# lmb-freiburg/hand3d

Hardware: NVIDIA H100
Metric: images/sec full pipeline 320x320 (higher is better)
Workload: dtype bf16 hi/lo split x3 MMA passes, fp32 accumulate (fp32 parity, 1e-3)

## Files before the change

### hand3d_b200/csrc/common.cuh

```cuda
#pragma once
#include <cuda_runtime.h>
#include <cuda_bf16.h>
#include <cuda_fp16.h>
#include <stdint.h>
#include <stdio.h>
#include <algorithm>
#include <cmath>
#include <string>
#include <vector>

#include "../../include/hand3d_b200.h"

namespace h3d {

void set_error(const char* fmt, ...);
int cuda_fail(cudaError_t e, const char* what, const char* file, int line);

#define H3D_CUDA(expr)                                                     \
    do {                                                                   \
        cudaError_t _e = (expr);                                           \
        if (_e != cudaSuccess) return h3d::cuda_fail(_e, #expr, __FILE__, __LINE__); \
    } while (0)

extern thread_local int64_t t_launches;
// ... 190 lines not shown
    int passes;
    float corr_scale = 0.f;
    Half16 half;
    int pool = 0;
    int* err_flag = nullptr;
    const int* count = nullptr;
};
struct TcTuning {
    int bn = 0;
    int chunk_kb = 0;
    int no_side_stream = 0, no_pool_fusion = 0, lift_direct = 0;
    int c3_ffma = 0;
    int no_seg_fusion = 0;
    int fc_chain = 1;
    int pdl = 1;
};
TcTuning& tc_tuning();
int tc_set_tuning(const char* key, int value);
struct FcLayerDesc {
    Split x; int x_stride, in_features;
    Split w; const float* bias; int out_features, out_pad;
    const float* w_scale = nullptr;
    Split y; int y_stride;
    float* yf; int yf_stride;
    int leaky;
};
struct FcChainDesc { FcLayerDesc layer[4]; int num_layers = 0; };
struct FcChainPlan;
FcChainPlan* fc_chain_plan_create(const FcChainDesc* chains, int num_chains, int B, Half16 half, const float* can, const float* uxyz,
                                  unsigned int* counter, int* err_flag);
void fc_chain_plan_destroy(FcChainPlan* p);
int fc_chain_launch(const FcChainPlan* p, const float* hand_side, float* rot, float* out, cudaStream_t s);
TcConvPlan* tc_conv_plan_create(const TcConvDesc& d, int* rc = nullptr);
void tc_conv_plan_destroy(TcConvPlan* p);
int tc_conv_launch(const TcConvPlan* p, cudaStream_t s);
int64_t tc_conv_flops(const TcConvPlan* p);
int tc_num_sms();
void tc_conv_geometry(int B, int H, int W, int Cout_pad, int pool, int passes, int out[4]);

int launch_pack_conv_w(const float* w_hwio, const float* bias, Split out, float* bias_pad, float* w_scale, int k, int Cin, int Cout,
                       int Cin_pad, int Cout_pad, bool dgrad, Half16 half, cudaStream_t s);
int conv_grad_prep_blocks(int64_t pixels, int64_t* pixels_per_block);
int launch_conv_grad_prep(const float* dy, const float* y, Split out, float* db_part, int B, int H, int W, int Cout, int Cout_pad,
                          int stride, int leaky, cudaStream_t s);
int launch_bias_grad_reduce(const float* db_part, int nblk, int Cout, int Cout_pad, float* db, cudaStream_t s);
struct WgradDesc {
    Split x;
    Split dy;
    int B, H, W, Cin, Cout, Cin_pad, Cout_pad, k, passes;
    float* partial;
    float* dw;
    int* err_flag;
};
// ... 32 lines not shown
```

### hand3d_b200/csrc/conv_wgmma.cu

```cuda
#include <cuda.h>

#include <algorithm>
#include <cstdlib>
#include <cstring>
#include <vector>

#include "common.cuh"
#include "split_fmt.cuh"
#include "wgmma_common.cuh"

namespace h3d {

namespace {

constexpr int BM = 128;
constexpr int BK = 64;
constexpr int kThreads = 384;
constexpr int kConsumerThreads = 256;
constexpr int A_TILE_BYTES = BM * BK * 2;
constexpr int STG_COLS = 64;
constexpr int STG_PITCH = STG_COLS + 1;
constexpr int STG_BYTES = BM * STG_PITCH * 4;
constexpr int kSmemBudget = 227 * 1024 - 2048 - STG_BYTES;

__host__ __device__ constexpr int stage_bytes(int BN, int PASSES) { return (PASSES >= 3 ? 2 : 1) * (A_TILE_BYTES + BN * BK * 2); }
__host__ __device__ constexpr int num_stages(int BN, int PASSES) {
    return kSmemBudget / stage_bytes(BN, PASSES) > 8 ? 8 : kSmemBudget / stage_bytes(BN, PASSES);
}
__host__ __device__ constexpr int smem_bytes(int BN, int PASSES) { return num_stages(BN, PASSES) * stage_bytes(BN, PASSES) + STG_BYTES + 2048; }

struct TcParams {
    const float* bias;
    uint16_t* y_hi; uint16_t* y_lo; uint8_t* y_l8; uint8_t* y_h8; int Cy_total, cy_off;
    float corr_scale;
    float* yf; int Cyf_total, cyf_off;
    int B, H, W, k, pad, cin_chunks;
    int TW, TH, TB, tiles_w, tiles_h, n_tiles, num_tiles;
    int n_valid;
    int pool;
    int chunk_kb;
    int leaky;
    int* err_flag;
    const float* w_scale;
    const int* count;
};

__device__ __forceinline__ int counted_images(const TcParams& p) { return p.count ? min(*p.count, p.B) : p.B; }
__device__ __forceinline__ int counted_tiles(const TcParams& p, int nb) {
    return p.count ? min(p.num_tiles, (nb + p.TB - 1) / p.TB * p.tiles_w * p.tiles_h * p.n_tiles) : p.num_tiles;
}

template <int PASSES, bool FP16, bool SMEM_SCALE = false>
__device__ __forceinline__ void epilogue_store32(const TcParams& p, const float* a, int64_t pix, int n, bool valid, const float* w_scale) {
    float f[32];
    const float4* bp = reinterpret_cast<const float4*>(p.bias + n);
#pragma unroll
    for (int q = 0; q < 8; ++q) {
        const float4 bv = __ldg(bp + q);
        if (PASSES == 4) {
            f[4 * q + 0] = fmaf(a[4 * q + 0], p.corr_scale, bv.x);
            f[4 * q + 1] = fmaf(a[4 * q + 1], p.corr_scale, bv.y);
            f[4 * q + 2] = fmaf(a[4 * q + 2], p.corr_scale, bv.z);
            f[4 * q + 3] = fmaf(a[4 * q + 3], p.corr_scale, bv.w);
        } else if (FP16) {
            const float4 sv = SMEM_SCALE ? reinterpret_cast<const float4*>(w_scale + n)[q] : __ldg(reinterpret_cast<const float4*>(w_scale + n) + q);
            f[4 * q + 0] = fmaf(a[4 * q + 0], sv.x, bv.x);
            f[4 * q + 1] = fmaf(a[4 * q + 1], sv.y, bv.y);
            f[4 * q + 2] = fmaf(a[4 * q + 2], sv.z, bv.z);
// ... 1 lines not shown
        } else {
            f[4 * q + 0] = a[4 * q + 0] + bv.x;
            f[4 * q + 1] = a[4 * q + 1] + bv.y;
            f[4 * q + 2] = a[4 * q + 2] + bv.z;
            f[4 * q + 3] = a[4 * q + 3] + bv.w;
        }
    }
    if (p.leaky) {
#pragma unroll
        for (int q = 0; q < 32; ++q) f[q] = fmaxf(f[q], kNegSlope * f[q]);
    }
    if (p.pool == 1) {
#pragma unroll
        for (int q = 0; q < 32; ++q) {
            f[q] = fmaxf(f[q], __shfl_xor_sync(0xFFFFFFFFu, f[q], 1));
            f[q] = fmaxf(f[q], __shfl_xor_sync(0xFFFFFFFFu, f[q], p.TW));
        }
    }
    if (!valid) return;
    if (n + 32 > p.n_valid) {
        const int cnt = p.n_valid - n;
        if (p.yf && cnt > 0) {
            float* dst = p.yf + pix * p.Cyf_total + p.cyf_off + n;
#pragma unroll
            for (int q = 0; q < 32; ++q)
                if (q < cnt) dst[q] = f[q];
        }
#pragma unroll
        for (int q = 0; q < 32; ++q)
            if (q >= cnt) f[q] = 0.f;
    } else if (p.yf) {
// ... 75 lines not shown
        if (PASSES == 3) {
            tma_load_4d(x_lo, st + A_TILE_BYTES, fb, a0, a1, a2, a3);
            tma_load_2d(w_lo, st + 2 * A_TILE_BYTES + C::B_TILE_BYTES, fb, kcol, n0);
        }
        if (PASSES == 4) {
            tma_load_4d(x_lo, st + A_TILE_BYTES, fb, a0, a1, a2, a3);
            tma_load_4d(x_h8, st + A_TILE_BYTES + C::A8_TILE_BYTES, fb, a0, a1, a2, a3);
            tma_load_2d(w_lo, st + 2 * A_TILE_BYTES + C::B_TILE_BYTES, fb, kcol, n0);
            tma_load_2d(w_l8, st + 2 * A_TILE_BYTES + C::B_TILE_BYTES + C::B8_TILE_BYTES, fb, kcol, n0);
        }
    }
    __syncwarp();
    if (++r.stage == C::STAGES) { r.stage = 0; r.phase ^= 1; }
}

template <int BN, int PASSES, bool FP16>
__device__ __forceinline__ void mma_tile(Ring& r, int kblocks, int chunk_kb, float* racc, int wg, int lane, int* err_flag) {
    using C = RingCfg<BN, PASSES>;
    constexpr int NR = BN / 2;
    constexpr int NR8 = PASSES == 4 ? NR : 1;
    float acc[NR], acc8[NR8];
#pragma unroll
    for (int i = 0; i < NR; ++i) acc[i] = 0.f;
#pragma unroll
    for (int i = 0; i < NR8; ++i) acc8[i] = 0.f;
    for (int kb0 = 0; kb0 < kblocks; kb0 += chunk_kb) {
        const int kb1 = min(kblocks, kb0 + chunk_kb);
        int pend = -1;
        for (int kb = kb0; kb < kb1; ++kb) {
            mbar_wait(&r.full[r.stage], r.phase, err_flag, 3);
            H3D_SKEW(SKEW_CONSUMER, kb);
            const uint32_t sa = smem_u32(r.base + r.stage * C::STAGE_BYTES);
            const uint32_t a_rows = (uint32_t)wg * 64 * 128;
            const uint64_t a_hi = desc_sw128(sa + a_rows);
            const uint64_t a_lo = desc_sw128(sa + A_TILE_BYTES + a_rows);
            const uint64_t b_hi = desc_sw128(sa + (PASSES >= 3 ? 2 : 1) * A_TILE_BYTES);
            const uint64_t b_lo = desc_sw128(sa + 2 * A_TILE_BYTES + C::B_TILE_BYTES);
            fence_regs<NR>(acc);
            fence_regs<NR8>(acc8);
            wgmma_fence();
#pragma unroll
            for (int j = 0; j < BK / 16; ++j) {
                const uint64_t koff = (uint64_t)j * 2;
                mma16<BN, FP16>(acc, a_hi + koff, b_hi + koff, (uint32_t)((kb > kb0) | (j != 0)));
                if (PASSES == 3) {
                    mma16<BN, FP16>(acc, a_hi + koff, b_lo + koff, 1u);
                    mma16<BN, FP16>(acc, a_lo + koff, b_hi + koff, 1u);
                }
            }
            if (PASSES == 4) {
                const uint32_t a8_rows = (uint32_t)wg * 64 * 64;
                const uint64_t a_l8 = desc_sw64(sa + A_TILE_BYTES + a8_rows);
// ... 2 lines not shown
                const uint64_t b_l8 = desc_sw64(sa + 2 * A_TILE_BYTES + C::B_TILE_BYTES + C::B8_TILE_BYTES);
#pragma unroll
                for (int j = 0; j < 2; ++j) {
                    const uint64_t koff = (uint64_t)j * 2;
                    mma8<BN>(acc8, a_l8 + koff, b_h8 + koff, (uint32_t)((kb > kb0) | (j != 0)));
                    mma8<BN>(acc8, a_h8 + koff, b_l8 + koff, 1u);
                }
            }
            wgmma_commit();
            fence_regs<NR>(acc);
            fence_regs<NR8>(acc8);
            H3D_SKEW(SKEW_COMMIT, kb);
            wgmma_wait<1>();
            if (pend >= 0 && lane == 0) mbar_arrive(&r.empty[pend]);
            pend = r.stage;
            if (++r.stage == C::STAGES) { r.stage = 0; r.phase ^= 1; }
        }
        wgmma_wait<0>();
        if (lane == 0) mbar_arrive(&r.empty[pend]);
        fence_regs<NR>(acc);
        fence_regs<NR8>(acc8);
        if constexpr (PASSES == 4) {
#pragma unroll
            for (int i = 0; i < NR; ++i) acc[i] += acc8[i];
        }
        if (kb0 == 0) {
#pragma unroll
            for (int i = 0; i < NR; ++i) racc[i] = acc[i];
        } else {
#pragma unroll
            for (int i = 0; i < NR; ++i) racc[i] += acc[i];
        }
    }
}

template <int BN, int PASSES, bool FP16, class PixOf, bool SMEM_SCALE = false>
__device__ __forceinline__ void store_tile(const TcParams& p, const float* racc, float* stg, int ct, int n0, PixOf pix_of,
                                           const float* w_scale) {
    const int wg = ct >> 7, tt = ct & 127;
    const int r0 = wg * 64 + (tt >> 5) * 16 + ((tt & 31) >> 2);
    const int cq = 2 * (tt & 3);
    const int row = ct & 127, half = ct >> 7;
    int64_t pix; bool valid;
    pix_of(row, pix, valid);
#pragma unroll
    for (int rnd = 0; rnd < BN / STG_COLS; ++rnd) {
        H3D_SKEW(SKEW_EPILOGUE, 2 * rnd);
        named_bar_sync(1, kConsumerThreads);
#pragma unroll
        for (int j = 0; j < STG_COLS / 8; ++j) {
            const int jj = rnd * (STG_COLS / 8) + j, c = 8 * j + cq;
            stg[r0 * STG_PITCH + c] = racc[4 * jj];
            stg[r0 * STG_PITCH + c + 1] = racc[4 * jj + 1];
            stg[(r0 + 8) * STG_PITCH + c] = racc[4 * jj + 2];
            stg[(r0 + 8) * STG_PITCH + c + 1] = racc[4 * jj + 3];
        }
        named_bar_sync(1, kConsumerThreads);
        H3D_SKEW(SKEW_EPILOGUE, 2 * rnd + 1);
        float f[32];
#pragma unroll
        for (int q = 0; q < 32; ++q) f[q] = stg[row * STG_PITCH + half * 32 + q];
        epilogue_store32<PASSES, FP16, SMEM_SCALE>(p, f, pix, n0 + rnd * STG_COLS + half * 32, valid, w_scale);
    }
}

constexpr int kProducerRegs = 40, kConsumerRegs = 232;

template <int BN, int PASSES, bool FP16>
__global__ void __launch_bounds__(kThreads, 1)
conv_tc_kernel(const __grid_constant__ CUtensorMap map_x_hi, const __grid_constant__ CUtensorMap map_x_lo,
               const __grid_constant__ CUtensorMap map_w_hi, const __grid_constant__ CUtensorMap map_w_lo,
               const __grid_constant__ CUtensorMap map_x_h8, const __grid_constant__ CUtensorMap map_w_l8, const TcParams p) {
    using C = RingCfg<BN, PASSES>;
    static_assert(PASSES != 4 || FP16, "fp8-correction mode uses an fp16 main plane");
    static_assert(smem_bytes(BN, PASSES) <= 227 * 1024, "conv_tc_kernel: shared memory budget");

    extern __shared__ __align__(1024) uint8_t smem_raw[];
    uint8_t* smem = reinterpret_cast<uint8_t*>((reinterpret_cast<uintptr_t>(smem_raw) + 1023) & ~(uintptr_t)1023);
    float* stg = reinterpret_cast<float*>(smem + C::STAGES * C::STAGE_BYTES);
    uint64_t* bars = reinterpret_cast<uint64_t*>(smem + C::STAGES * C::STAGE_BYTES + STG_BYTES);
    Ring ring{smem, bars, bars + C::STAGES, 0, 0};

    const int warp = threadIdx.x >> 5, lane = threadIdx.x & 31;
    const int wg = __shfl_sync(0xFFFFFFFFu, (int)threadIdx.x / 128, 0);
    const int kblocks = p.k * p.k * p.cin_chunks;

    if (threadIdx.x == 0) {
        prefetch_tmap(&map_x_hi); prefetch_tmap(&map_w_hi);
        if (PASSES >= 3) { prefetch_tmap(&map_x_lo); prefetch_tmap(&map_w_lo); }
        if (PASSES == 4) { prefetch_tmap(&map_x_h8); prefetch_tmap(&map_w_l8); }
        for (int s = 0; s < C::STAGES; ++s) { mbar_init(&ring.full[s], 1); mbar_init(&ring.empty[s], kConsumerThreads / 32); }
        asm volatile("fence.mbarrier_init.release.cluster;" ::: "memory");
    }
    __syncthreads();
    pdl_launch_dependents();
    H3D_SKEW(SKEW_PDL_TAIL, 0);
    pdl_wait();
    const int nb = counted_images(p), num_tiles = counted_tiles(p, nb);

    if (wg == 0) {
        setmaxnreg_dec<kProducerRegs>();
        if (warp == 0) {
            for (int tile = blockIdx.x; tile < num_tiles; tile += gridDim.x) {
                const int nt = tile % p.n_tiles, mt = tile / p.n_tiles;
                const int tw = mt % p.tiles_w, th = (mt / p.tiles_w) % p.tiles_h, tb = mt / (p.tiles_w * p.tiles_h);
                const int w0 = tw * p.TW - p.pad, h0 = th * p.TH - p.pad, b0 = tb * p.TB, n0 = nt * BN;
                int kcol = 0;
                for (int kh = 0; kh < p.k; ++kh)
                    for (int kw = 0; kw < p.k; ++kw)
                        for (int cc = 0; cc < p.cin_chunks; ++cc, kcol += BK)
                            produce_kblock<BN, PASSES>(ring, &map_x_hi, &map_x_lo, &map_x_h8, &map_w_hi, &map_w_lo, &map_w_l8, cc * BK,
                                                       w0 + kw, h0 + kh, b0, kcol, n0, p.err_flag);
            }
        }
    } else {
        setmaxnreg_inc<kConsumerRegs>();
        const int ct = threadIdx.x - 128;
        float racc[BN / 2];
        for (int tile = blockIdx.x; tile < num_tiles; tile += gridDim.x) {
            const int nt = tile % p.n_tiles, mt = tile / p.n_tiles;
            const int tw = mt % p.tiles_w, th = (mt / p.tiles_w) % p.tiles_h, tb = mt / (p.tiles_w * p.tiles_h);
            mma_tile<BN, PASSES, FP16>(ring, kblocks, p.chunk_kb, racc, ct >> 7, lane, p.err_flag);
            store_tile<BN, PASSES, FP16>(p, racc, stg, ct, nt * BN, [&](int row, int64_t& pix, bool& valid) {
                const int w_l = row % p.TW, h_l = (row / p.TW) % p.TH, b_l = row / (p.TW * p.TH);
                const int w = tw * p.TW + w_l, h = th * p.TH + h_l, b = tb * p.TB + b_l;
                valid = (w < p.W) && (h < p.H) && (b < nb);
                pix = ((int64_t)b * p.H + h) * p.W + w;
                if (p.pool) {
                    const int par = p.pool == 2 ? 1 : 0;
                    valid = valid && ((w & 1) == par) && ((h & 1) == par);
                    pix = ((int64_t)b * (p.H >> 1) + (h >> 1)) * (p.W >> 1) + (w >> 1);
                }
            }, p.w_scale);
        }
    }
}

constexpr int C3_TW = 16, C3_TH = 8;
constexpr int C3T_THREADS = 256;
constexpr int C3T_B_BYTES = 128 * BK * 2;
constexpr int C3T_PW = C3_TW + 2, C3T_PH = C3_TH + 2;
constexpr int C3T_PATCH_FLOATS = C3T_PH * C3T_PW * 3;
constexpr int C3T_SMEM = C3T_B_BYTES + 2 * A_TILE_BYTES + STG_BYTES + C3T_PATCH_FLOATS * 4 + 64 * 4 + 1024 ;

template <bool FP16, bool COUNTED>
__global__ void __launch_bounds__(C3T_THREADS, 2)
conv_c3_tc_kernel(const float* __restrict__ x, const float* __restrict__ w, const TcParams p, const int* __restrict__ slots) {
    extern __shared__ __align__(1024) uint8_t smem_raw[];
    uint8_t* smem = reinterpret_cast<uint8_t*>((reinterpret_cast<uintptr_t>(smem_raw) + 1023) & ~(uintptr_t)1023);
    uint8_t* bsm = smem;
// ... 78 lines not shown
        for (int j = 0; j < 2; ++j) {
            const uint64_t koff = (uint64_t)j * 2;
            mma16<64, FP16>(acc, a_hi + koff, b_hi + koff, (uint32_t)(j != 0));
            mma16<64, FP16>(acc, a_hi + koff, b_lo + koff, 1u);
            mma16<64, FP16>(acc, a_lo + koff, b_hi + koff, 1u);
        }
        wgmma_commit();
        H3D_SKEW(SKEW_COMMIT, tile);
        wgmma_wait<0>();
        fence_regs<32>(acc);
        auto pix_of = [&](int row, int64_t& pix, bool& valid) {
            const int wx = tw * C3_TW + row % C3_TW, hy = th * C3_TH + row / C3_TW;
            valid = (wx < p.W) && (hy < p.H);
            pix = ((int64_t)b * p.H + hy) * p.W + wx;
        };
        if (p.y_lo) store_tile<64, 3, FP16, decltype(pix_of), true>(p, acc, stg, t, 0, pix_of, w_scale);
        else store_tile<64, 1, FP16, decltype(pix_of), true>(p, acc, stg, t, 0, pix_of, w_scale);
    }
}

constexpr int kFcMaxLayers = 4;
constexpr int kFcCluster = 8;
struct FcLayer {
    CUtensorMap map_x_hi, map_x_lo, map_w_hi, map_w_lo;
    TcParams p;
    int kblocks, m_tiles, n_tiles, pad_;
};
struct FcChain { FcLayer layer[kFcMaxLayers]; int num_layers; int pad_[3]; };
struct FcChainParams {
    FcChain chain[2];
    int num_chains, B;
    const float* can; const float* uxyz; const float* hand_side;
// ... 48 lines not shown
            for (int item = rank; item < items; item += kFcCluster) {
                const int nt = item % L.n_tiles, mt = item / L.n_tiles;
                for (int kb = 0; kb < L.kblocks; ++kb)
                    produce_kblock<BN, PASSES>(ring, &L.map_x_hi, &L.map_x_lo, &L.map_x_hi, &L.map_w_hi, &L.map_w_lo, &L.map_w_hi, kb * BK, 0, 0,
                                               mt * BM, kb * BK, nt * BN, P.err_flag);
            }
        } else if (wg >= 1) {
            const int ct = threadIdx.x - 128;
            float racc[BN / 2];
            for (int item = rank; item < items; item += kFcCluster) {
                const int nt = item % L.n_tiles, mt = item / L.n_tiles;
                mma_tile<BN, PASSES, FP16>(ring, L.kblocks, kChunk, racc, ct >> 7, lane, P.err_flag);
                store_tile<BN, PASSES, FP16>(L.p, racc, stg, ct, nt * BN, [&](int row, int64_t& pix, bool& valid) {
                    pix = (int64_t)mt * BM + row;
                    valid = pix < P.B;
                }, L.p.w_scale);
            }
        }
        fc_layer_sync(l);
    }

    if (P.num_chains == 2 && rank == 0) {
        H3D_SKEW(SKEW_TICKET, 0);
        if (threadIdx.x == 0) {
            __threadfence();
            s_last = atomicAdd(P.counter, 1u) == 1u;
            if (s_last) *P.counter = 0u;
        }
        __syncthreads();
        if (s_last) {
            __threadfence();
// ... 41 lines not shown

bool encode_act_map(CUtensorMap* m, const void* base, int C_total, int C_used, int W, int H, int B, int TW, int TH, int TB, int es) {
    EncodeTiledFn fn = get_encode_fn();
    if (!fn) return false;
    cuuint64_t dims[4] = {(cuuint64_t)C_used, (cuuint64_t)W, (cuuint64_t)H, (cuuint64_t)B};
    cuuint64_t strides[3] = {(cuuint64_t)C_total * es, (cuuint64_t)W * C_total * es, (cuuint64_t)H * W * C_total * es};
    cuuint32_t box[4] = {(cuuint32_t)BK, (cuuint32_t)TW, (cuuint32_t)TH, (cuuint32_t)TB};
    cuuint32_t estr[4] = {1, 1, 1, 1};
    CUresult r = fn(m, es == 2 ? CU_TENSOR_MAP_DATA_TYPE_UINT16 : CU_TENSOR_MAP_DATA_TYPE_UINT8, 4, const_cast<void*>(base), dims, strides,
                    box, estr, CU_TENSOR_MAP_INTERLEAVE_NONE, es == 2 ? CU_TENSOR_MAP_SWIZZLE_128B : CU_TENSOR_MAP_SWIZZLE_64B,
                    CU_TENSOR_MAP_L2_PROMOTION_L2_256B, CU_TENSOR_MAP_FLOAT_OOB_FILL_NONE);
    if (r != CUDA_SUCCESS) { set_error("cuTensorMapEncodeTiled(activations) failed: %d", (int)r); return false; }
    return true;
}

bool encode_w_map(CUtensorMap* m, const void* base, int Ktot, int Cout_pad, int BN, int es) {
    EncodeTiledFn fn = get_encode_fn();
    if (!fn) return false;
    cuuint64_t dims[2] = {(cuuint64_t)Ktot, (cuuint64_t)Cout_pad};
    cuuint64_t strides[1] = {(cuuint64_t)Ktot * es};
    cuuint32_t box[2] = {(cuuint32_t)BK, (cuuint32_t)BN};
    cuuint32_t estr[2] = {1, 1};
    CUresult r = fn(m, es == 2 ? CU_TENSOR_MAP_DATA_TYPE_UINT16 : CU_TENSOR_MAP_DATA_TYPE_UINT8, 2, const_cast<void*>(base), dims, strides,
                    box, estr, CU_TENSOR_MAP_INTERLEAVE_NONE, es == 2 ? CU_TENSOR_MAP_SWIZZLE_128B : CU_TENSOR_MAP_SWIZZLE_64B,
                    CU_TENSOR_MAP_L2_PROMOTION_L2_256B, CU_TENSOR_MAP_FLOAT_OOB_FILL_NONE);
    if (r != CUDA_SUCCESS) { set_error("cuTensorMapEncodeTiled(weights) failed: %d", (int)r); return false; }
    return true;
}

namespace {

void choose_tile(int B, int H, int W, int* TW, int* TH, int* TB, bool pool = false) {
    static const int cand[][3] = {{16, 8, 1}, {8, 16, 1}, {32, 4, 1}, {4, 32, 1}, {64, 2, 1}, {128, 1, 1}, {8, 8, 2},
                                  {16, 4, 2}, {4, 16, 2}, {8, 4, 4}, {4, 8, 4}, {4, 4, 8}, {8, 2, 8}, {2, 2, 32}, {1, 1, 128}};
    int64_t best = -1;
    for (auto& c : cand) {
        if (pool && !((c[0] % 2) == 0 && c[0] <= 16 && (c[1] % 2) == 0)) continue;
        const int64_t tiles = (int64_t)ceil_div(W, c[0]) * ceil_div(H, c[1]) * ceil_div(B, c[2]);
        if (best < 0 || tiles < best) { best = tiles; *TW = c[0]; *TH = c[1]; *TB = c[2]; }
    }
}

template <int BN, int PASSES, bool FP16>
int launch_inst(const TcConvPlan* pl, cudaStream_t s);

}

struct TcConvPlan {
    int device = 0;
    TcConvDesc d;
    CUtensorMap map_x_hi, map_x_lo, map_w_hi, map_w_lo, map_x_h8, map_w_l8;
    TcParams p;
    int BN, grid;
};

constexpr int kMaxDevices = 64;
static int current_device() { int dev = 0; if (cudaGetDevice(&dev) != cudaSuccess) { cudaGetLastError(); dev = 0; } return dev; }
int tc_num_sms() {
    static int n[kMaxDevices] = {};
    const int dev = current_device() % kMaxDevices;
    if (!n[dev]) {
        int v = 0;
        if (cudaDeviceGetAttribute(&v, cudaDevAttrMultiProcessorCount, dev) != cudaSuccess || v <= 0) { cudaGetLastError(); v = 132; }
        n[dev] = v;
    }
    return n[dev];
}
template <typename K>
// ... 60 lines not shown
}
#endif

int tc_set_tuning(const char* key, int value) {
    TcTuning& t = tc_tuning();
    const std::string k(key ? key : "");
    if (k == "tc_bn") t.bn = value;
    else if (k == "tc_chunk_kb") t.chunk_kb = value;
    else if (k == "no_side_stream") t.no_side_stream = value;
    else if (k == "no_pool_fusion") t.no_pool_fusion = value;
    else if (k == "lift_direct") t.lift_direct = value;
    else if (k == "c3_ffma") t.c3_ffma = value;
    else if (k == "pdl") t.pdl = value;
    else if (k == "fc_chain") t.fc_chain = value;
    else if (k == "no_seg_fusion") t.no_seg_fusion = value;
#ifdef H3D_SKEW_BUILD
    else if (k.compare(0, 5, "skew_") == 0) return skew_set(key, value);
#endif
    else { set_error("h3d_set_tuning: unknown key '%s'", k.c_str()); return H3D_EINVAL; }
    return H3D_OK;
}

namespace {
int choose_bn(int H, int W, int Cout_pad, int passes) {
    const TcTuning& tune = tc_tuning();
    int BN = Cout_pad % 128 == 0 ? 128 : 64;
    if ((int64_t)H * W <= 256) BN = 64;
    if ((tune.bn == 64 || tune.bn == 128) && Cout_pad % tune.bn == 0) BN = tune.bn;
    if (passes == 4) BN = 64;
    return BN;
}

template <int BN, int PASSES, bool FP16>
int launch_inst(const TcConvPlan* pl, cudaStream_t s) {
    constexpr int smem = smem_bytes(BN, PASSES);
    static bool attr[kMaxDevices] = {};
    if (int rc = smem_opt_in(conv_tc_kernel<BN, PASSES, FP16>, smem, attr)) return rc;
    H3D_CUDA(launch_pdl(conv_tc_kernel<BN, PASSES, FP16>, dim3(pl->grid), dim3(kThreads), smem, s, pl->map_x_hi, pl->map_x_lo, pl->map_w_hi,
                        pl->map_w_lo, pl->map_x_h8, pl->map_w_l8, pl->p));
    return H3D_OK;
}
}

TcConvPlan* tc_conv_plan_create(const TcConvDesc& d, int* rc) {
    int rc_local;
    if (!rc) rc = &rc_local;
    *rc = H3D_EINVAL;
    if (d.Cin_pad % BK != 0 || d.Cout_pad % 64 != 0 || (d.k != 1 && d.k != 3 && d.k != 5 && d.k != 7) || (d.passes != 1 && d.passes != 3 && d.passes != 4)) {
        set_error("tc_conv: unsupported geometry (Cin_pad=%d Cout_pad=%d k=%d passes=%d)", d.Cin_pad, d.Cout_pad, d.k, d.passes);
        return nullptr;
    }
    const bool padded_out = d.Cout % 32 != 0;
    if (d.y.hi && ((d.Cy_total % 8) || (d.cy_off % 8))) { set_error("tc_conv: split output channel offset/stride must be multiples of 8"); return nullptr; }
    if (d.yf && !padded_out && ((d.Cyf_total % 4) || (d.cyf_off % 4))) { set_error("tc_conv: fp32 output channel offset/stride must be multiples of 4"); return nullptr; }
// ... 25 lines not shown
    p.yf = d.yf; p.Cyf_total = d.Cyf_total; p.cyf_off = d.cyf_off;
    p.B = d.B; p.H = d.H; p.W = d.W; p.k = d.k; p.pad = d.k / 2; p.cin_chunks = d.Cin_pad / BK;
    p.TW = TW; p.TH = TH; p.TB = TB;
    p.tiles_w = ceil_div(d.W, TW); p.tiles_h = ceil_div(d.H, TH);
    p.n_tiles = d.Cout_pad / BN;
    p.num_tiles = p.tiles_w * p.tiles_h * ceil_div(d.B, TB) * p.n_tiles;
    p.leaky = d.leaky;
    p.n_valid = d.Cout;
    p.pool = d.pool;
    p.err_flag = d.err_flag;
    p.w_scale = d.w_scale;
    p.count = d.count;
    p.chunk_kb = d.passes >= 3 ? 9 : 27;
    if (tune.chunk_kb > 0) p.chunk_kb = tune.chunk_kb;
    pl->grid = std::min(p.num_tiles, tc_num_sms());
    const int Ktot = d.k * d.k * d.Cin_pad;
    bool ok = encode_act_map(&pl->map_x_hi, d.x.hi, d.Cin_total, d.Cin_pad, d.W, d.H, d.B, TW, TH, TB) &&
              encode_w_map(&pl->map_w_hi, d.w.hi, Ktot, d.Cout_pad, BN);
    if (ok && d.passes == 3)
        ok = encode_act_map(&pl->map_x_lo, d.x.lo, d.Cin_total, d.Cin_pad, d.W, d.H, d.B, TW, TH, TB) &&
             encode_w_map(&pl->map_w_lo, d.w.lo, Ktot, d.Cout_pad, BN);
    if (ok && d.passes == 4)
        ok = encode_act_map(&pl->map_x_lo, d.x.l8, d.Cin_total, d.Cin_pad, d.W, d.H, d.B, TW, TH, TB, 1) &&
             encode_act_map(&pl->map_x_h8, d.x.h8, d.Cin_total, d.Cin_pad, d.W, d.H, d.B, TW, TH, TB, 1) &&
             encode_w_map(&pl->map_w_lo, d.w.h8, Ktot, d.Cout_pad, BN, 1) &&
             encode_w_map(&pl->map_w_l8, d.w.l8, Ktot, d.Cout_pad, BN, 1);
    if (ok && d.passes == 1) { pl->map_x_lo = pl->map_x_hi; pl->map_w_lo = pl->map_w_hi; }
    if (ok && d.passes != 4) { pl->map_x_h8 = pl->map_x_hi; pl->map_w_l8 = pl->map_w_hi; }
    if (!ok) { delete pl; return nullptr; }
    *rc = H3D_OK;
    return pl;
}

void tc_conv_plan_destroy(TcConvPlan* p) { delete p; }

void tc_conv_geometry(int B, int H, int W, int Cout_pad, int pool, int passes, int out[4]) {
    choose_tile(B, H, W, &out[0], &out[1], &out[2], pool == 1);
    out[3] = choose_bn(H, W, Cout_pad, passes);
}

int64_t tc_conv_flops(const TcConvPlan* p) {
    return 2ll * p->d.B * p->d.H * p->d.W * p->d.k * p->d.k * (int64_t)p->d.Cin_pad * p->d.Cout_pad;
}

int tc_conv_launch(const TcConvPlan* pl, cudaStream_t s) {
    const bool fp16 = pl->d.half == Half16::FP16;
    const int key = pl->BN * 10 + pl->d.passes;
#define CASE(BN_, P_)                                                                  \
    case BN_ * 10 + P_:                                                                \
        return fp16 ? launch_inst<BN_, P_, true>(pl, s) : launch_inst<BN_, P_, false>(pl, s);
    switch (key) {
        CASE(64, 1) CASE(64, 3) CASE(128, 1) CASE(128, 3)
        case 64 * 10 + 4: return launch_inst<64, 4, true>(pl, s);
    }
#undef CASE
    set_error("tc_conv: no kernel instance for BN=%d passes=%d", pl->BN, pl->d.passes);
    return H3D_EINVAL;
}

int launch_conv_c3_tc(const float* x, const float* w, const float* bias, Split y, int Cs_total, int cs_off, int B, int H, int W, int leaky,
                      Half16 half, cudaStream_t s, int* err_flag, const int* count, const int* slots) {
    H3D_REQUIRE(x && w && bias && y.hi && !y.l8 && (Cs_total % 8) == 0 && (cs_off % 8) == 0, "conv_c3_tc: bad argument");
    TcParams p{};
    p.bias = bias;
    p.y_hi = y.hi; p.y_lo = y.lo; p.Cy_total = Cs_total; p.cy_off = cs_off;
    p.corr_scale = 1.f;
    p.B = B; p.H = H; p.W = W; p.k = 3; p.pad = 1; p.cin_chunks = 1;
    p.TW = C3_TW; p.TH = C3_TH; p.TB = 1;
// ... 72 lines not shown
```

### hand3d_b200/runtime.py

```python
from __future__ import annotations

import ctypes as C

import numpy as np
import torch

from . import _lib
from ._lib import PRECISIONS, VARIANTS


def _ptr(t):
    return C.c_void_p(0 if t is None else t.data_ptr())


def _stream():
    return C.c_void_p(torch.cuda.current_stream().cuda_stream)


def _chk_f32(t, name, ndim=None):
    if not isinstance(t, torch.Tensor):
        raise TypeError("%s must be a torch.Tensor" % name)
    if not t.is_cuda:
        raise RuntimeError("%s must live on a CUDA device (hand3d_b200 has no CPU path)" % name)
    if t.dtype != torch.float32:
# ... 1080 lines not shown
        B = self.B
        self.center = self.buffer[_lib.TRACK_CENTER * B:(_lib.TRACK_CENTER + 2) * B].view(B, 2)
        self.scale = self.buffer[_lib.TRACK_SCALE * B:(_lib.TRACK_SCALE + 1) * B]
        self.score = self.buffer[_lib.TRACK_SCORE * B:(_lib.TRACK_SCORE + 1) * B]
        self.lost = self.buffer[_lib.TRACK_LOST * B:(_lib.TRACK_LOST + 1) * B].view(torch.int32)
        self.reset()

    def reset(self):
        self.center.fill_(160.0)
        self.scale.fill_(float(np.float32(256.0) / (np.float32(100.0) * np.float32(1.25))))
        self.score.fill_(float("nan"))
        self.lost.fill_(1)


def conv2d_tc_geometry(B, H, W, Cout, pool=0, precision="bf16x3"):
    out = (C.c_int * 4)()
    _lib.check(_lib.load().h3d_conv2d_tc_geometry(B, H, W, Cout, int(pool), PRECISIONS[precision], out), "h3d_conv2d_tc_geometry")
    return tuple(out)


def conv2d_wgrad_geometry(B, H, W, ksize, Cin, Cout):
    out = (C.c_int * 6)()
    _lib.check(_lib.load().h3d_conv2d_wgrad_geometry(B, H, W, ksize, Cin, Cout, out), "h3d_conv2d_wgrad_geometry")
    return tuple(out)


def conv2d_f32_geometry(B, H, W, Cin, Cout, ksize, stride=1, Cin_total=None, cin_off=0, Cout_total=None, cout_off=0, yf=True,
                        planes=None, Cs_total=None, cs_off=0, x_aligned=True, splitk_scratch_floats=_lib.CONV_SPLITK_SCRATCH_FLOATS):
    out = (C.c_int * 6)()
    _lib.check(_lib.load().h3d_conv2d_f32_geometry(
        B, H, W, Cin, Cin if Cin_total is None else Cin_total, cin_off, Cout, Cout if Cout_total is None else Cout_total, cout_off,
# ... 24 lines not shown
```

Measured before the change: 1259.

## Feed conv activations as one TMA row box reused across kernel columns

Adds a row-box feed path to the implicit-GEMM conv kernel. For each kernel row it loads one wide activation box (TW+k-1 columns) and reuses it for all k horizontal taps by offsetting the smem descriptor, while weights stream through a separate ring. The goal is fewer activation TMA loads and less duplicated smem traffic for k>=3 layers with a single 64-channel input chunk. In exchange the pixel ordering within a tile changes (h-major), the pooling shuffle offset changes, and a second barrier ring plus a runtime-sized smem layout are added.

```diff
diff --git a/hand3d_b200/csrc/common.cuh b/hand3d_b200/csrc/common.cuh
--- a/hand3d_b200/csrc/common.cuh
+++ b/hand3d_b200/csrc/common.cuh
@@ -228,6 +228,7 @@
     int no_seg_fusion = 0;
     int fc_chain = 1;
     int pdl = 1;
+    int feed = 0;
 };
 TcTuning& tc_tuning();
 int tc_set_tuning(const char* key, int value);
@@ -250,7 +251,7 @@
 int tc_conv_launch(const TcConvPlan* p, cudaStream_t s);
 int64_t tc_conv_flops(const TcConvPlan* p);
 int tc_num_sms();
-void tc_conv_geometry(int B, int H, int W, int Cout_pad, int pool, int passes, int out[4]);
+void tc_conv_geometry(int B, int H, int W, int Cout_pad, int pool, int passes, int out[5]);
 
 int launch_pack_conv_w(const float* w_hwio, const float* bias, Split out, float* bias_pad, float* w_scale, int k, int Cin, int Cout,
                        int Cin_pad, int Cout_pad, bool dgrad, Half16 half, cudaStream_t s);
diff --git a/hand3d_b200/csrc/conv_wgmma.cu b/hand3d_b200/csrc/conv_wgmma.cu
--- a/hand3d_b200/csrc/conv_wgmma.cu
+++ b/hand3d_b200/csrc/conv_wgmma.cu
@@ -28,6 +28,9 @@
     return kSmemBudget / stage_bytes(BN, PASSES) > 8 ? 8 : kSmemBudget / stage_bytes(BN, PASSES);
 }
 __host__ __device__ constexpr int smem_bytes(int BN, int PASSES) { return num_stages(BN, PASSES) * stage_bytes(BN, PASSES) + STG_BYTES + 2048; }
+constexpr int kRowSlots = 2;
+constexpr int kMaxWStages = 8;
+__host__ __device__ constexpr int wstage_bytes(int BN, int PASSES) { return (PASSES >= 3 ? 2 : 1) * BN * BK * 2; }
 
 struct TcParams {
     const float* bias;
@@ -43,6 +46,7 @@
     int* err_flag;
     const float* w_scale;
     const int* count;
+    int box_bytes, w_stages, wg_rows;
 };
 
 __device__ __forceinline__ int counted_images(const TcParams& p) { return p.count ? min(*p.count, p.B) : p.B; }
@@ -51,7 +55,8 @@
 }
 
 template <int PASSES, bool FP16, bool SMEM_SCALE = false>
-__device__ __forceinline__ void epilogue_store32(const TcParams& p, const float* a, int64_t pix, int n, bool valid, const float* w_scale) {
+__device__ __forceinline__ void epilogue_store32(const TcParams& p, const float* a, int64_t pix, int n, bool valid, int pool_xor,
+                                                 const float* w_scale) {
     float f[32];
     const float4* bp = reinterpret_cast<const float4*>(p.bias + n);
 #pragma unroll
@@ -83,7 +88,7 @@
 #pragma unroll
         for (int q = 0; q < 32; ++q) {
             f[q] = fmaxf(f[q], __shfl_xor_sync(0xFFFFFFFFu, f[q], 1));
-            f[q] = fmaxf(f[q], __shfl_xor_sync(0xFFFFFFFFu, f[q], p.TW));
+            f[q] = fmaxf(f[q], __shfl_xor_sync(0xFFFFFFFFu, f[q], pool_xor));
         }
     }
     if (!valid) return;
@@ -189,28 +194,88 @@
     if (++r.stage == C::STAGES) { r.stage = 0; r.phase ^= 1; }
 }
 
-template <int BN, int PASSES, bool FP16>
-__device__ __forceinline__ void mma_tile(Ring& r, int kblocks, int chunk_kb, float* racc, int wg, int lane, int* err_flag) {
+struct RowFeed {
+    Ring a;
+    int k, box_bytes, w_stages;
+    uint32_t wg_off, kw_off;
+};
+
+template <int PASSES>
+__device__ __forceinline__ void produce_box(RowFeed& f, const CUtensorMap* x_hi, const CUtensorMap* x_lo, int h, int w, int b, int* err_flag) {
+    Ring& r = f.a;
+    mbar_wait(&r.empty[r.stage], r.phase ^ 1, err_flag, 1);
+    H3D_SKEW(SKEW_PRODUCER, r.stage + r.phase * kRowSlots);
+    if (elect_one()) {
+        uint8_t* st = r.base + r.stage * (PASSES == 3 ? 2 : 1) * f.box_bytes;
+        uint64_t* fb = &r.full[r.stage];
+        mbar_expect_tx(fb, (PASSES == 3 ? 2 : 1) * f.box_bytes);
+        tma_load_4d(x_hi, st, fb, 0, h, w, b);
+        if (PASSES == 3) tma_load_4d(x_lo, st + f.box_bytes, fb, 0, h, w, b);
+    }
+    __syncwarp();
+    if (++r.stage == kRowSlots) { r.stage = 0; r.phase ^= 1; }
+}
+
+template <int BN, int PASSES>
+__device__ __forceinline__ void produce_wblock(Ring& r, int w_stages, const CUtensorMap* w_hi, const CUtensorMap* w_lo, int kcol, int n0,
+                                               int* err_flag) {
     using C = RingCfg<BN, PASSES>;
+    mbar_wait(&r.empty[r.stage], r.phase ^ 1, err_flag, 1);
+    H3D_SKEW(SKEW_PRODUCER, r.stage + r.phase * w_stages);
+    if (elect_one()) {
+        uint8_t* st = r.base + r.stage * wstage_bytes(BN, PASSES);
+        uint64_t* fb = &r.full[r.stage];
+        mbar_expect_tx(fb, wstage_bytes(BN, PASSES));
+        tma_load_2d(w_hi, st, fb, kcol, n0);
+        if (PASSES == 3) tma_load_2d(w_lo, st + C::B_TILE_BYTES, fb, kcol, n0);
+    }
+    __syncwarp();
+    if (++r.stage == w_stages) { r.stage = 0; r.phase ^= 1; }
+}
+
+template <int BN, int PASSES, bool FP16, bool ROW_BOX = false>
+__device__ __forceinline__ void mma_tile(Ring& r, int kblocks, int chunk_kb, float* racc, int wg, int lane, int* err_flag,
+                                         RowFeed* f = nullptr) {
+    using C = RingCfg<BN, PASSES>;
+    static_assert(!ROW_BOX || PASSES != 4, "the row-box feed has 16-bit planes only");
     constexpr int NR = BN / 2;
     constexpr int NR8 = PASSES == 4 ? NR : 1;
+    const int stages = ROW_BOX ? f->w_stages : C::STAGES;
     float acc[NR], acc8[NR8];
 #pragma unroll
     for (int i = 0; i < NR; ++i) acc[i] = 0.f;
 #pragma unroll
     for (int i = 0; i < NR8; ++i) acc8[i] = 0.f;
+    int kw = 0;
     for (int kb0 = 0; kb0 < kblocks; kb0 += chunk_kb) {
         const int kb1 = min(kblocks, kb0 + chunk_kb);
-        int pend = -1;
+        int pend = -1, pend_box = -1;
         for (int kb = kb0; kb < kb1; ++kb) {
-            mbar_wait(&r.full[r.stage], r.phase, err_flag, 3);
-            H3D_SKEW(SKEW_CONSUMER, kb);
-            const uint32_t sa = smem_u32(r.base + r.stage * C::STAGE_BYTES);
-            const uint32_t a_rows = (uint32_t)wg * 64 * 128;
-            const uint64_t a_hi = desc_sw128(sa + a_rows);
-            const uint64_t a_lo = desc_sw128(sa + A_TILE_BYTES + a_rows);
-            const uint64_t b_hi = desc_sw128(sa + (PASSES >= 3 ? 2 : 1) * A_TILE_BYTES);
-            const uint64_t b_lo = desc_sw128(sa + 2 * A_TILE_BYTES + C::B_TILE_BYTES);
+            uint64_t a_hi, a_lo, b_hi, b_lo;
+            uint32_t sa = 0;
+            if constexpr (ROW_BOX) {
+                if (kw == 0) {
+                    mbar_wait(&f->a.full[f->a.stage], f->a.phase, err_flag, 3);
+                    H3D_SKEW(SKEW_CONSUMER, kb);
+                }
+                mbar_wait(&r.full[r.stage], r.phase, err_flag, 3);
+                H3D_SKEW(SKEW_CONSUMER, kb);
+                const uint32_t box = smem_u32(f->a.base + f->a.stage * (PASSES == 3 ? 2 : 1) * f->box_bytes) + wg * f->wg_off + kw * f->kw_off;
+                const uint32_t sb = smem_u32(r.base + r.stage * wstage_bytes(BN, PASSES));
+                a_hi = desc_sw128(box);
+                a_lo = desc_sw128(box + f->box_bytes);
+                b_hi = desc_sw128(sb);
+                b_lo = desc_sw128(sb + C::B_TILE_BYTES);
+            } else {
+                mbar_wait(&r.full[r.stage], r.phase, err_flag, 3);
+                H3D_SKEW(SKEW_CONSUMER, kb);
+                sa = smem_u32(r.base + r.stage * C::STAGE_BYTES);
+                const uint32_t a_rows = (uint32_t)wg * 64 * 128;
+                a_hi = desc_sw128(sa + a_rows);
+                a_lo = desc_sw128(sa + A_TILE_BYTES + a_rows);
+                b_hi = desc_sw128(sa + (PASSES >= 3 ? 2 : 1) * A_TILE_BYTES);
+                b_lo = desc_sw128(sa + 2 * A_TILE_BYTES + C::B_TILE_BYTES);
+            }
             fence_regs<NR>(acc);
             fence_regs<NR8>(acc8);
             wgmma_fence();
@@ -243,10 +308,22 @@
             wgmma_wait<1>();
             if (pend >= 0 && lane == 0) mbar_arrive(&r.empty[pend]);
             pend = r.stage;
-            if (++r.stage == C::STAGES) { r.stage = 0; r.phase ^= 1; }
+            if (++r.stage == stages) { r.stage = 0; r.phase ^= 1; }
+            if constexpr (ROW_BOX) {
+                if (pend_box >= 0 && lane == 0) mbar_arrive(&f->a.empty[pend_box]);
+                pend_box = -1;
+                if (++kw == f->k) {
+                    kw = 0;
+                    pend_box = f->a.stage;
+                    if (++f->a.stage == kRowSlots) { f->a.stage = 0; f->a.phase ^= 1; }
+                }
+            }
         }
         wgmma_wait<0>();
         if (lane == 0) mbar_arrive(&r.empty[pend]);
+        if constexpr (ROW_BOX) {
+            if (pend_box >= 0 && lane == 0) mbar_arrive(&f->a.empty[pend_box]);
+        }
         fence_regs<NR>(acc);
         fence_regs<NR8>(acc8);
         if constexpr (PASSES == 4) {
@@ -264,7 +341,7 @@
 }
 
 template <int BN, int PASSES, bool FP16, class PixOf, bool SMEM_SCALE = false>
-__device__ __forceinline__ void store_tile(const TcParams& p, const float* racc, float* stg, int ct, int n0, PixOf pix_of,
+__device__ __forceinline__ void store_tile(const TcParams& p, const float* racc, float* stg, int ct, int n0, PixOf pix_of, int pool_xor,
                                            const float* w_scale) {
     const int wg = ct >> 7, tt = ct & 127;
     const int r0 = wg * 64 + (tt >> 5) * 16 + ((tt & 31) >> 2);
@@ -289,26 +366,29 @@
         float f[32];
 #pragma unroll
         for (int q = 0; q < 32; ++q) f[q] = stg[row * STG_PITCH + half * 32 + q];
-        epilogue_store32<PASSES, FP16, SMEM_SCALE>(p, f, pix, n0 + rnd * STG_COLS + half * 32, valid, w_scale);
+        epilogue_store32<PASSES, FP16, SMEM_SCALE>(p, f, pix, n0 + rnd * STG_COLS + half * 32, valid, pool_xor, w_scale);
     }
 }
 
 constexpr int kProducerRegs = 40, kConsumerRegs = 232;
 
-template <int BN, int PASSES, bool FP16>
-__global__ void __launch_bounds__(kThreads, 1)
-conv_tc_kernel(const __grid_constant__ CUtensorMap map_x_hi, const __grid_constant__ CUtensorMap map_x_lo,
-               const __grid_constant__ CUtensorMap map_w_hi, const __grid_constant__ CUtensorMap map_w_lo,
-               const __grid_constant__ CUtensorMap map_x_h8, const __grid_constant__ CUtensorMap map_w_l8, const TcParams p) {
+template <int BN, int PASSES, bool FP16, bool ROW_BOX>
+__device__ __forceinline__ void conv_tc_body(const CUtensorMap& map_x_hi, const CUtensorMap& map_x_lo, const CUtensorMap& map_w_hi,
+                                             const CUtensorMap& map_w_lo, const CUtensorMap& map_x_h8, const CUtensorMap& map_w_l8,
+                                             const TcParams& p) {
     using C = RingCfg<BN, PASSES>;
     static_assert(PASSES != 4 || FP16, "fp8-correction mode uses an fp16 main plane");
     static_assert(smem_bytes(BN, PASSES) <= 227 * 1024, "conv_tc_kernel: shared memory budget");
 
     extern __shared__ __align__(1024) uint8_t smem_raw[];
     uint8_t* smem = reinterpret_cast<uint8_t*>((reinterpret_cast<uintptr_t>(smem_raw) + 1023) & ~(uintptr_t)1023);
-    float* stg = reinterpret_cast<float*>(smem + C::STAGES * C::STAGE_BYTES);
-    uint64_t* bars = reinterpret_cast<uint64_t*>(smem + C::STAGES * C::STAGE_BYTES + STG_BYTES);
-    Ring ring{smem, bars, bars + C::STAGES, 0, 0};
+    const int stages = ROW_BOX ? p.w_stages : C::STAGES;
+    uint8_t* wring = ROW_BOX ? smem + kRowSlots * (PASSES == 3 ? 2 : 1) * p.box_bytes : smem;
+    float* stg = reinterpret_cast<float*>(wring + (ROW_BOX ? p.w_stages * wstage_bytes(BN, PASSES) : C::STAGES * C::STAGE_BYTES));
+    uint64_t* bars = reinterpret_cast<uint64_t*>(reinterpret_cast<uint8_t*>(stg) + STG_BYTES);
+    Ring ring{wring, bars, bars + stages, 0, 0};
+    RowFeed feed{{smem, bars + 2 * stages, bars + 2 * stages + kRowSlots, 0, 0}, p.k, p.box_bytes, p.w_stages,
+                 (uint32_t)p.wg_rows * 128, (uint32_t)p.TH * 128};
 
     const int warp = threadIdx.x >> 5, lane = threadIdx.x & 31;
     const int wg = __shfl_sync(0xFFFFFFFFu, (int)threadIdx.x / 128, 0);
@@ -318,7 +398,9 @@
         prefetch_tmap(&map_x_hi); prefetch_tmap(&map_w_hi);
         if (PASSES >= 3) { prefetch_tmap(&map_x_lo); prefetch_tmap(&map_w_lo); }
         if (PASSES == 4) { prefetch_tmap(&map_x_h8); prefetch_tmap(&map_w_l8); }
-        for (int s = 0; s < C::STAGES; ++s) { mbar_init(&ring.full[s], 1); mbar_init(&ring.empty[s], kConsumerThreads / 32); }
+        for (int s = 0; s < stages; ++s) { mbar_init(&ring.full[s], 1); mbar_init(&ring.empty[s], kConsumerThreads / 32); }
+        if (ROW_BOX)
+            for (int s = 0; s < kRowSlots; ++s) { mbar_init(&feed.a.full[s], 1); mbar_init(&feed.a.empty[s], kConsumerThreads / 32); }
         asm volatile("fence.mbarrier_init.release.cluster;" ::: "memory");
     }
     __syncthreads();
@@ -335,11 +417,18 @@
                 const int tw = mt % p.tiles_w, th = (mt / p.tiles_w) % p.tiles_h, tb = mt / (p.tiles_w * p.tiles_h);
                 const int w0 = tw * p.TW - p.pad, h0 = th * p.TH - p.pad, b0 = tb * p.TB, n0 = nt * BN;
                 int kcol = 0;
-                for (int kh = 0; kh < p.k; ++kh)
-                    for (int kw = 0; kw < p.k; ++kw)
-                        for (int cc = 0; cc < p.cin_chunks; ++cc, kcol += BK)
-                            produce_kblock<BN, PASSES>(ring, &map_x_hi, &map_x_lo, &map_x_h8, &map_w_hi, &map_w_lo, &map_w_l8, cc * BK,
-                                                       w0 + kw, h0 + kh, b0, kcol, n0, p.err_flag);
+                for (int kh = 0; kh < p.k; ++kh) {
+                    if constexpr (ROW_BOX) {
+                        produce_box<PASSES>(feed, &map_x_hi, &map_x_lo, h0 + kh, w0, b0, p.err_flag);
+                        for (int kw = 0; kw < p.k; ++kw, kcol += BK)
+                            produce_wblock<BN, PASSES>(ring, stages, &map_w_hi, &map_w_lo, kcol, n0, p.err_flag);
+                    } else {
+                        for (int kw = 0; kw < p.k; ++kw)
+                            for (int cc = 0; cc < p.cin_chunks; ++cc, kcol += BK)
+                                produce_kblock<BN, PASSES>(ring, &map_x_hi, &map_x_lo, &map_x_h8, &map_w_hi, &map_w_lo, &map_w_l8, cc * BK,
+                                                           w0 + kw, h0 + kh, b0, kcol, n0, p.err_flag);
+                    }
+                }
             }
         }
     } else {
@@ -349,9 +438,11 @@
         for (int tile = blockIdx.x; tile < num_tiles; tile += gridDim.x) {
             const int nt = tile % p.n_tiles, mt = tile / p.n_tiles;
             const int tw = mt % p.tiles_w, th = (mt / p.tiles_w) % p.tiles_h, tb = mt / (p.tiles_w * p.tiles_h);
-            mma_tile<BN, PASSES, FP16>(ring, kblocks, p.chunk_kb, racc, ct >> 7, lane, p.err_flag);
+            mma_tile<BN, PASSES, FP16, ROW_BOX>(ring, kblocks, p.chunk_kb, racc, ct >> 7, lane, p.err_flag, &feed);
             store_tile<BN, PASSES, FP16>(p, racc, stg, ct, nt * BN, [&](int row, int64_t& pix, bool& valid) {
-                const int w_l = row % p.TW, h_l = (row / p.TW) % p.TH, b_l = row / (p.TW * p.TH);
+                const int w_l = ROW_BOX ? (row / p.TH) % p.TW : row % p.TW;
+                const int h_l = ROW_BOX ? row % p.TH : (row / p.TW) % p.TH;
+                const int b_l = row / (p.TW * p.TH);
                 const int w = tw * p.TW + w_l, h = th * p.TH + h_l, b = tb * p.TB + b_l;
                 valid = (w < p.W) && (h < p.H) && (b < nb);
                 pix = ((int64_t)b * p.H + h) * p.W + w;
@@ -360,9 +451,24 @@
                     valid = valid && ((w & 1) == par) && ((h & 1) == par);
                     pix = ((int64_t)b * (p.H >> 1) + (h >> 1)) * (p.W >> 1) + (w >> 1);
                 }
-            }, p.w_scale);
-        }
-    }
+            }, ROW_BOX ? p.TH : p.TW, p.w_scale);
+        }
+    }
+}
+
+template <int BN, int PASSES, bool FP16>
+__global__ void __launch_bounds__(kThreads, 1)
+conv_tc_kernel(const __grid_constant__ CUtensorMap map_x_hi, const __grid_constant__ CUtensorMap map_x_lo,
+               const __grid_constant__ CUtensorMap map_w_hi, const __grid_constant__ CUtensorMap map_w_lo,
+               const __grid_constant__ CUtensorMap map_x_h8, const __grid_constant__ CUtensorMap map_w_l8, const __grid_constant__ TcParams p) {
+    conv_tc_body<BN, PASSES, FP16, false>(map_x_hi, map_x_lo, map_w_hi, map_w_lo, map_x_h8, map_w_l8, p);
+}
+template <int BN, int PASSES, bool FP16>
+__global__ void __launch_bounds__(kThreads, 1)
+conv_tc_kernel_rowbox(const __grid_constant__ CUtensorMap map_x_hi, const __grid_constant__ CUtensorMap map_x_lo,
+                      const __grid_constant__ CUtensorMap map_w_hi, const __grid_constant__ CUtensorMap map_w_lo,
+                      const __grid_constant__ CUtensorMap map_x_h8, const __grid_constant__ CUtensorMap map_w_l8, const __grid_constant__ TcParams p) {
+    conv_tc_body<BN, PASSES, FP16, true>(map_x_hi, map_x_lo, map_w_hi, map_w_lo, map_x_h8, map_w_l8, p);
 }
 
 constexpr int C3_TW = 16, C3_TH = 8;
@@ -471,8 +577,8 @@
             valid = (wx < p.W) && (hy < p.H);
             pix = ((int64_t)b * p.H + hy) * p.W + wx;
         };
-        if (p.y_lo) store_tile<64, 3, FP16, decltype(pix_of), true>(p, acc, stg, t, 0, pix_of, w_scale);
-        else store_tile<64, 1, FP16, decltype(pix_of), true>(p, acc, stg, t, 0, pix_of, w_scale);
+        if (p.y_lo) store_tile<64, 3, FP16, decltype(pix_of), true>(p, acc, stg, t, 0, pix_of, C3_TW, w_scale);
+        else store_tile<64, 1, FP16, decltype(pix_of), true>(p, acc, stg, t, 0, pix_of, C3_TW, w_scale);
     }
 }
 
@@ -551,7 +657,7 @@
                 store_tile<BN, PASSES, FP16>(L.p, racc, stg, ct, nt * BN, [&](int row, int64_t& pix, bool& valid) {
                     pix = (int64_t)mt * BM + row;
                     valid = pix < P.B;
-                }, L.p.w_scale);
+                }, L.p.TW, L.p.w_scale);
             }
         }
         fc_layer_sync(l);
@@ -623,6 +729,19 @@
     return true;
 }
 
+static bool encode_row_box_map(CUtensorMap* m, const void* base, int C_total, int C_used, int W, int H, int B, int TW, int TH, int TB, int k) {
+    EncodeTiledFn fn = get_encode_fn();
+    if (!fn) return false;
+    cuuint64_t dims[4] = {(cuuint64_t)C_used, (cuuint64_t)H, (cuuint64_t)W, (cuuint64_t)B};
+    cuuint64_t strides[3] = {(cuuint64_t)W * C_total * 2, (cuuint64_t)C_total * 2, (cuuint64_t)H * W * C_total * 2};
+    cuuint32_t box[4] = {(cuuint32_t)BK, (cuuint32_t)TH, (cuuint32_t)(TW + k - 1), (cuuint32_t)TB};
+    cuuint32_t estr[4] = {1, 1, 1, 1};
+    CUresult r = fn(m, CU_TENSOR_MAP_DATA_TYPE_UINT16, 4, const_cast<void*>(base), dims, strides, box, estr, CU_TENSOR_MAP_INTERLEAVE_NONE,
+                    CU_TENSOR_MAP_SWIZZLE_128B, CU_TENSOR_MAP_L2_PROMOTION_L2_256B, CU_TENSOR_MAP_FLOAT_OOB_FILL_NONE);
+    if (r != CUDA_SUCCESS) { set_error("cuTensorMapEncodeTiled(row-box activations) failed: %d", (int)r); return false; }
+    return true;
+}
+
 bool encode_w_map(CUtensorMap* m, const void* base, int Ktot, int Cout_pad, int BN, int es) {
     EncodeTiledFn fn = get_encode_fn();
     if (!fn) return false;
@@ -650,7 +769,19 @@
     }
 }
 
-template <int BN, int PASSES, bool FP16>
+int row_box_stages(int k, int cin_chunks, int passes, int pool, int TW, int TH, int TB, int BN, int* box_bytes) {
+    *box_bytes = 0;
+    if (tc_tuning().feed == 1 || k < 3 || cin_chunks != 1 || (passes != 1 && passes != 3) || TH % 8 != 0 ||
+        (TB != 1 && TW * TH != 64) || (pool == 1 && TH > 16))
+        return 0;
+    const int plane = TB * (TW + k - 1) * TH * 128;
+    const int slots = kRowSlots * (passes == 3 ? 2 : 1) * plane, ws = wstage_bytes(BN, passes);
+    if (slots + 3 * ws > kSmemBudget) return 0;
+    *box_bytes = plane;
+    return std::min(kMaxWStages, (kSmemBudget - slots) / ws);
+}
+
+template <int BN, int PASSES, bool FP16, bool ROW_BOX>
 int launch_inst(const TcConvPlan* pl, cudaStream_t s);
 
 }
@@ -660,7 +791,7 @@
     TcConvDesc d;
     CUtensorMap map_x_hi, map_x_lo, map_w_hi, map_w_lo, map_x_h8, map_w_l8;
     TcParams p;
-    int BN, grid;
+    int BN, grid, smem;
 };
 
 constexpr int kMaxDevices = 64;
@@ -751,6 +882,7 @@
     else if (k == "pdl") t.pdl = value;
     else if (k == "fc_chain") t.fc_chain = value;
     else if (k == "no_seg_fusion") t.no_seg_fusion = value;
+    else if (k == "tc_feed") t.feed = value;
 #ifdef H3D_SKEW_BUILD
     else if (k.compare(0, 5, "skew_") == 0) return skew_set(key, value);
 #endif
@@ -768,13 +900,15 @@
     return BN;
 }
 
-template <int BN, int PASSES, bool FP16>
+template <int BN, int PASSES, bool FP16, bool ROW_BOX>
 int launch_inst(const TcConvPlan* pl, cudaStream_t s) {
-    constexpr int smem = smem_bytes(BN, PASSES);
+    constexpr int smem_max = ROW_BOX ? 227 * 1024 : smem_bytes(BN, PASSES);
+    auto* kernel = conv_tc_kernel<BN, PASSES, FP16>;
+    if constexpr (ROW_BOX) kernel = conv_tc_kernel_rowbox<BN, PASSES, FP16>;
     static bool attr[kMaxDevices] = {};
-    if (int rc = smem_opt_in(conv_tc_kernel<BN, PASSES, FP16>, smem, attr)) return rc;
-    H3D_CUDA(launch_pdl(conv_tc_kernel<BN, PASSES, FP16>, dim3(pl->grid), dim3(kThreads), smem, s, pl->map_x_hi, pl->map_x_lo, pl->map_w_hi,
-                        pl->map_w_lo, pl->map_x_h8, pl->map_w_l8, pl->p));
+    if (int rc = smem_opt_in(kernel, smem_max, attr)) return rc;
+    H3D_CUDA(launch_pdl(kernel, dim3(pl->grid), dim3(kThreads), pl->smem, s, pl->map_x_hi, pl->map_x_lo,
+                        pl->map_w_hi, pl->map_w_lo, pl->map_x_h8, pl->map_w_l8, pl->p));
     return H3D_OK;
 }
 }
@@ -830,12 +964,18 @@
     p.chunk_kb = d.passes >= 3 ? 9 : 27;
     if (tune.chunk_kb > 0) p.chunk_kb = tune.chunk_kb;
     pl->grid = std::min(p.num_tiles, tc_num_sms());
+    p.w_stages = row_box_stages(d.k, p.cin_chunks, d.passes, d.pool, TW, TH, TB, BN, &p.box_bytes);
+    p.wg_rows = TB == 1 ? 64 : TH * (TW + d.k - 1);
+    const bool row_box = p.w_stages > 0;
+    pl->smem = row_box ? kRowSlots * (d.passes == 3 ? 2 : 1) * p.box_bytes + p.w_stages * wstage_bytes(BN, d.passes) + STG_BYTES + 2048
+                       : smem_bytes(BN, d.passes);
+    auto act_map = [&](CUtensorMap* m, const void* x) {
+        return row_box ? encode_row_box_map(m, x, d.Cin_total, d.Cin_pad, d.W, d.H, d.B, TW, TH, TB, d.k)
+                       : encode_act_map(m, x, d.Cin_total, d.Cin_pad, d.W, d.H, d.B, TW, TH, TB);
+    };
     const int Ktot = d.k * d.k * d.Cin_pad;
-    bool ok = encode_act_map(&pl->map_x_hi, d.x.hi, d.Cin_total, d.Cin_pad, d.W, d.H, d.B, TW, TH, TB) &&
-              encode_w_map(&pl->map_w_hi, d.w.hi, Ktot, d.Cout_pad, BN);
-    if (ok && d.passes == 3)
-        ok = encode_act_map(&pl->map_x_lo, d.x.lo, d.Cin_total, d.Cin_pad, d.W, d.H, d.B, TW, TH, TB) &&
-             encode_w_map(&pl->map_w_lo, d.w.lo, Ktot, d.Cout_pad, BN);
+    bool ok = act_map(&pl->map_x_hi, d.x.hi) && encode_w_map(&pl->map_w_hi, d.w.hi, Ktot, d.Cout_pad, BN);
+    if (ok && d.passes == 3) ok = act_map(&pl->map_x_lo, d.x.lo) && encode_w_map(&pl->map_w_lo, d.w.lo, Ktot, d.Cout_pad, BN);
     if (ok && d.passes == 4)
         ok = encode_act_map(&pl->map_x_lo, d.x.l8, d.Cin_total, d.Cin_pad, d.W, d.H, d.B, TW, TH, TB, 1) &&
              encode_act_map(&pl->map_x_h8, d.x.h8, d.Cin_total, d.Cin_pad, d.W, d.H, d.B, TW, TH, TB, 1) &&
@@ -850,9 +990,12 @@
 
 void tc_conv_plan_destroy(TcConvPlan* p) { delete p; }
 
-void tc_conv_geometry(int B, int H, int W, int Cout_pad, int pool, int passes, int out[4]) {
+void tc_conv_geometry(int B, int H, int W, int Cout_pad, int pool, int passes, int out[5]) {
     choose_tile(B, H, W, &out[0], &out[1], &out[2], pool == 1);
     out[3] = choose_bn(H, W, Cout_pad, passes);
+    out[4] = 0;
+    for (int k = 3, box; k <= 7; k += 2)
+        if (row_box_stages(k, 1, passes, pool, out[0], out[1], out[2], out[3], &box)) out[4] = k;
 }
 
 int64_t tc_conv_flops(const TcConvPlan* p) {
@@ -862,12 +1005,13 @@
 int tc_conv_launch(const TcConvPlan* pl, cudaStream_t s) {
     const bool fp16 = pl->d.half == Half16::FP16;
     const int key = pl->BN * 10 + pl->d.passes;
-#define CASE(BN_, P_)                                                                  \
-    case BN_ * 10 + P_:                                                                \
-        return fp16 ? launch_inst<BN_, P_, true>(pl, s) : launch_inst<BN_, P_, false>(pl, s);
+#define CASE(BN_, P_)                                                                                                       \
+    case BN_ * 10 + P_:                                                                                                     \
+        if (pl->p.w_stages) return fp16 ? launch_inst<BN_, P_, true, true>(pl, s) : launch_inst<BN_, P_, false, true>(pl, s); \
+        return fp16 ? launch_inst<BN_, P_, true, false>(pl, s) : launch_inst<BN_, P_, false, false>(pl, s);
     switch (key) {
         CASE(64, 1) CASE(64, 3) CASE(128, 1) CASE(128, 3)
-        case 64 * 10 + 4: return launch_inst<64, 4, true>(pl, s);
+        case 64 * 10 + 4: return launch_inst<64, 4, true, false>(pl, s);
     }
 #undef CASE
     set_error("tc_conv: no kernel instance for BN=%d passes=%d", pl->BN, pl->d.passes);
diff --git a/hand3d_b200/runtime.py b/hand3d_b200/runtime.py
--- a/hand3d_b200/runtime.py
+++ b/hand3d_b200/runtime.py
@@ -1118,7 +1118,15 @@
 
 
 def conv2d_tc_geometry(B, H, W, Cout, pool=0, precision="bf16x3"):
-    out = (C.c_int * 4)()
+    return _conv2d_tc_geometry(B, H, W, Cout, pool, precision)[:4]
+
+
+def conv2d_tc_row_box(B, H, W, Cin, Cout, ksize, pool=0, precision="bf16x3"):
+    return Cin <= 64 and ksize >= 3 and ksize <= _conv2d_tc_geometry(B, H, W, Cout, pool, precision)[4]
+
+
+def _conv2d_tc_geometry(B, H, W, Cout, pool, precision):
+    out = (C.c_int * 5)()
     _lib.check(_lib.load().h3d_conv2d_tc_geometry(B, H, W, Cout, int(pool), PRECISIONS[precision], out), "h3d_conv2d_tc_geometry")
     return tuple(out)
 
```

Result: no change. 1268 (median of 6 runs) (+0.7%).
